# kohjingyu/gill

Hardware: AMD Instinct MI355X
Metric: 512x512 images/sec/node, OPT-6.7B+SD1.5 50-step (higher is better)
Workload: dtype bf16

## Files before the change

gill_amd/csrc/attention.hip:

```cpp
#include "ops.h"
#include <stdlib.h>
#include <type_traits>

#define ATT_KVT 64

template <int DP, int ATT_THREADS>
struct AttCfg {
  static constexpr int KS = DP / 16;
  static constexpr int NDT = (DP + 31) / 32;
  static constexpr int DPV = NDT * 32;
  static constexpr int KSTR = DP + 8;
  static constexpr int VSTR = ATT_KVT + 8;
  static constexpr bool HAS_ONES = (DP % 32) != 0;
  static constexpr int K_CHUNKS = ATT_KVT * DP / 8;
  static constexpr int V_CHUNKS = DPV * ATT_KVT / 8;
  static constexpr int K_PER_THR = (K_CHUNKS + ATT_THREADS - 1) / ATT_THREADS;
  static constexpr int V_PER_THR = (V_CHUNKS + ATT_THREADS - 1) / ATT_THREADS;
  static constexpr int K_ROWS = (K_PER_THR * ATT_THREADS + DP / 8 - 1) / (DP / 8);
  static constexpr int V_ROWS = K_PER_THR * 0 + V_PER_THR * ATT_THREADS / 8;
  static constexpr int K_ELEMS = K_ROWS * KSTR;
  static constexpr int V_ELEMS = V_ROWS * VSTR;
  static constexpr int BUF_ELEMS = K_ELEMS + V_ELEMS;
  static constexpr int SMEM_BYTES = 2 * BUF_ELEMS * 2;
};

template <int DP, int ATT_THREADS>
__global__ __launch_bounds__(ATT_THREADS, (DP <= 64 ? 4 : 2)) void attention_kernel(const AttnArgs p) {
  kernarg_warm<sizeof(AttnArgs)>();
  using Cfg = AttCfg<DP, ATT_THREADS>;
  constexpr int ATT_QB = ATT_THREADS / 2;
  constexpr int KS = Cfg::KS, NDT = Cfg::NDT, KSTR = Cfg::KSTR, VSTR = Cfg::VSTR;
  extern __shared__ __attribute__((aligned(16))) unsigned char att_smem_raw[];
  bf16_t* smem = reinterpret_cast<bf16_t*>(att_smem_raw);

  const int tid = threadIdx.x;
  const int lane = tid & 63;
  const int w = tid >> 6;
  const int nqt = (p.nq + ATT_QB - 1) / ATT_QB;
  int pair, qtile;
  if (p.xcd_map) {
    const int xcd = blockIdx.x & 7, slot = blockIdx.x >> 3;
    pair = xcd + 8 * (slot / nqt);
    qtile = slot - (slot / nqt) * nqt;
  } else {
    pair = blockIdx.x / nqt;
    qtile = blockIdx.x - pair * nqt;
  }
  if (pair >= p.B * p.H) return;
  const int b = pair / p.H, h = pair - b * p.H;
  const int q0 = qtile * ATT_QB + w * 32;
  const bool wave_active = q0 < p.nq;
  const int lq = lane & 31;
  const int hi = lane >> 5;
  const int kvb = p.kv_bstride_zero ? 0 : b;

  const bf16_t* Qb = p.Q + (size_t)(b * p.H + h) * p.nq_pad * DP;
  const bf16_t* Kb = p.K + (size_t)(kvb * p.H + h) * p.nkv_pad * DP;
  const bf16_t* Vb = p.Vt + (size_t)(kvb * p.H + h) * p.dpv * p.nkv_pad;

  int qrow = q0 + lq;
  const bool qvalid = qrow < p.nq;
  if (qrow > p.nq - 1) qrow = p.nq - 1;

  bf16x8 qf[KS];
#pragma unroll
  for (int s = 0; s < KS; ++s) qf[s] = *reinterpret_cast<const bf16x8*>(Qb + (size_t)qrow * DP + s * 16 + hi * 8);

  f32x16 oacc[NDT];
#pragma unroll
  for (int t = 0; t < NDT; ++t)
#pragma unroll
    for (int r = 0; r < 16; ++r) oacc[t][r] = 0.f;

  float m_run = 0.f, l_run = 0.f;

  const int coff = p.nkv - p.nq;
  int kv_end_blk = p.nkv;
  if (p.causal) {
    int lim = qtile * ATT_QB + ATT_QB - 1 + coff + 1;
    if (lim < kv_end_blk) kv_end_blk = lim;
    if (kv_end_blk < 1) kv_end_blk = 1;
  }
  const int ntiles = (kv_end_blk + ATT_KVT - 1) / ATT_KVT;
  const int qidx = qrow + coff;
  const int wave_kv_end = p.causal ? min(p.nkv, q0 + 31 + coff + 1) : p.nkv;

  typedef __attribute__((ext_vector_type(4))) unsigned int u32x4;
  u32x4 kreg[Cfg::K_PER_THR];
  u32x4 vreg[Cfg::V_PER_THR];
  auto gload = [&](int tile) {
    const int kv0 = tile * ATT_KVT;
#pragma unroll
    for (int i = 0; i < Cfg::K_PER_THR; ++i) {
      int c = tid + i * ATT_THREADS;
      if (c > Cfg::K_CHUNKS - 1) c = Cfg::K_CHUNKS - 1;
      int row = c / (DP / 8);
      const int col = c - row * (DP / 8);
      if (kv0 + row > p.nkv_pad - 1) row = p.nkv_pad - 1 - kv0;
      kreg[i] = *reinterpret_cast<const u32x4*>(Kb + (size_t)(kv0 + row) * DP + col * 8);
    }
#pragma unroll
    for (int i = 0; i < Cfg::V_PER_THR; ++i) {
      int c = tid + i * ATT_THREADS;
      if (c > Cfg::V_CHUNKS - 1) c = Cfg::V_CHUNKS - 1;
      const int row = c >> 3;
      int col = (c & 7) * 8;
      if (kv0 + col > p.nkv_pad - 8) col = p.nkv_pad - 8 - kv0;
      vreg[i] = *reinterpret_cast<const u32x4*>(Vb + (size_t)row * p.nkv_pad + kv0 + col);
    }
  };
  auto lstore = [&](int buf) {
    bf16_t* Ks = smem + buf * Cfg::BUF_ELEMS;
    bf16_t* Vs = Ks + Cfg::K_ELEMS;
#pragma unroll
    for (int i = 0; i < Cfg::K_PER_THR; ++i) {
      const int c = tid + i * ATT_THREADS;
      const int row = c / (DP / 8);
      const int col = c - row * (DP / 8);
      *reinterpret_cast<u32x4*>(Ks + row * KSTR + col * 8) = kreg[i];
    }
#pragma unroll
    for (int i = 0; i < Cfg::V_PER_THR; ++i) {
      const int c = tid + i * ATT_THREADS;
      const int row = c >> 3;
      const int col = (c & 7) * 8;
      bf16_t* d = Vs + row * VSTR + (col & ~15) + ((col & 8) >> 1);
      *reinterpret_cast<uint2*>(d) = make_uint2(vreg[i][0], vreg[i][1]);
      *reinterpret_cast<uint2*>(d + 8) = make_uint2(vreg[i][2], vreg[i][3]);
    }
  };

  const int rot = (p.causal || !p.xcd_map) ? 0 : (qtile * 5) % ntiles;
  gload(rot);
  lstore(0);
  __syncthreads();

  for (int it = 0; it < ntiles; ++it) {
    int tile = it + rot;
    if (tile >= ntiles) tile -= ntiles;
    const int kv0 = tile * ATT_KVT;
    if (it + 1 < ntiles) gload(tile + 1 < ntiles ? tile + 1 : 0);
    const bf16_t* Ks = smem + (it & 1) * Cfg::BUF_ELEMS;
    const bf16_t* Vs = Ks + Cfg::K_ELEMS;

    if (wave_active && kv0 < wave_kv_end) {
      const bool first = (it == 0);
      const float acc0 = first ? 0.f : -m_run;
      f32x16 s[2];
#pragma unroll
      for (int hh = 0; hh < 2; ++hh) {
#pragma unroll
        for (int r = 0; r < 16; ++r) s[hh][r] = acc0;
        const bf16_t* krow = Ks + (hh * 32 + lq) * KSTR + hi * 8;
#pragma unroll
        for (int ks = 0; ks < KS; ++ks) {
          const bf16x8 kf = *reinterpret_cast<const bf16x8*>(krow + ks * 16);
          s[hh] = __builtin_amdgcn_mfma_f32_32x32x16_bf16(kf, qf[ks], s[hh], 0, 0, 0);
        }
      }
      const bool need_mask = (kv0 + ATT_KVT > p.nkv) || (p.causal && (kv0 + ATT_KVT - 1 > q0 + coff));
      if (need_mask) {
#pragma unroll
        for (int hh = 0; hh < 2; ++hh)
#pragma unroll
          for (int r = 0; r < 16; ++r) {
            const int kv = kv0 + hh * 32 + (r & 3) + 8 * (r >> 2) + 4 * hi;
            const bool masked = (kv >= p.nkv) || (p.causal && kv > qidx);
            s[hh][r] = masked ? -INFINITY : s[hh][r];
          }
      }
      float mx = s[0][0];
#pragma unroll
      for (int hh = 0; hh < 2; ++hh)
#pragma unroll
        for (int r = 0; r < 16; ++r) mx = fmaxf(mx, s[hh][r]);
      mx = fmaxf(mx, __shfl_xor(mx, 32, 64));
      const bool grow = first || (mx > 8.0f);
      if (__any(grow)) {
        float delta;
        if (first) { m_run = (mx > -INFINITY) ? mx : 0.f; delta = m_run; }
        else { delta = grow ? mx : 0.f; m_run += delta; }
        if (!first) {
          const float alpha = __builtin_amdgcn_exp2f(-delta);
          l_run *= alpha;
#pragma unroll
          for (int t = 0; t < NDT; ++t)
#pragma unroll
            for (int r = 0; r < 16; ++r) oacc[t][r] *= alpha;
        }
#pragma unroll
        for (int hh = 0; hh < 2; ++hh)
#pragma unroll
          for (int r = 0; r < 16; ++r) s[hh][r] -= delta;
      }
#pragma unroll
      for (int hh = 0; hh < 2; ++hh)
#pragma unroll
        for (int r = 0; r < 16; ++r) s[hh][r] = __builtin_amdgcn_exp2f(s[hh][r]);
      if constexpr (!Cfg::HAS_ONES) {
        float rs = 0.f;
#pragma unroll
        for (int hh = 0; hh < 2; ++hh)
#pragma unroll
          for (int r = 0; r < 16; ++r) rs += s[hh][r];
        rs += __shfl_xor(rs, 32, 64);
        l_run += rs;
      }

      bf16x8 pa[4];
#pragma unroll
      for (int h4 = 0; h4 < 4; ++h4) {
        union { bf16x8 v; uint32_t u[4]; } pk;
#pragma unroll
        for (int j = 0; j < 4; ++j) pk.u[j] = pack_bf2(s[h4 >> 1][(h4 & 1) * 8 + 2 * j], s[h4 >> 1][(h4 & 1) * 8 + 2 * j + 1]);
        pa[h4] = pk.v;
      }
#pragma unroll
      for (int t = 0; t < NDT; ++t) {
        const bf16_t* vrow = Vs + (t * 32 + lq) * VSTR + 8 * hi;
#pragma unroll
        for (int h4 = 0; h4 < 4; ++h4) {
          const bf16x8 vf = *reinterpret_cast<const bf16x8*>(vrow + 16 * h4);
          oacc[t] = __builtin_amdgcn_mfma_f32_32x32x16_bf16(vf, pa[h4], oacc[t], 0, 0, 0);
        }
      }
    }
    if (it + 1 < ntiles) lstore((it + 1) & 1);
    __syncthreads();
  }

  if (!wave_active) return;
  if constexpr (Cfg::HAS_ONES) {
    static_assert(DP % 32 == 16, "ones-row position");
    l_run = __shfl(oacc[DP / 32][8], lq, 64);
  }
  if (!qvalid) return;
  const float inv = 1.f / l_run;
  bf16_t* orow = p.O + (size_t)(b * p.nq + qrow) * p.ldo + h * DP;
#pragma unroll
  for (int t = 0; t < NDT; ++t) {
#pragma unroll
    for (int g = 0; g < 4; ++g) {
      const int d = t * 32 + 8 * g + 4 * hi;
      if (d < DP) {
        uint2 o;
        o.x = pack_bf2(oacc[t][g * 4 + 0] * inv, oacc[t][g * 4 + 1] * inv);
        o.y = pack_bf2(oacc[t][g * 4 + 2] * inv, oacc[t][g * 4 + 3] * inv);
        *reinterpret_cast<uint2*>(orow + d) = o;
      }
    }
  }
}


template <int DP, int ATT_THREADS>
__global__ __launch_bounds__(ATT_THREADS, 4) void attention_dma_kernel(const AttnArgs p) {
  kernarg_warm<sizeof(AttnArgs)>();
  static_assert(DP == 48, "QF3 needs three padding dims behind d = 40");
  constexpr int NW = ATT_THREADS / 64;
  constexpr int ATT_QB = ATT_THREADS / 2;
  constexpr int KS = DP / 16, NDT = (DP + 31) / 32, NCH = DP / 8;
  constexpr int PPW = 8 / NW;
  constexpr int K_BYTES = 64 * 128, STAGE = 2 * K_BYTES, CONST_OFF = 2 * STAGE;
  extern __shared__ __attribute__((aligned(16))) unsigned char att_smem_raw[];
  unsigned char* smem = att_smem_raw;

  const int tid = threadIdx.x;
  const int lane = tid & 63;
  const int w = __builtin_amdgcn_readfirstlane(tid >> 6);
  const int nqt = p.nq / ATT_QB;
  int pair, qtile;
  if (p.xcd_map) {
    const int xcd = blockIdx.x & 7, slot = blockIdx.x >> 3;
    pair = xcd + 8 * (slot / nqt);
    qtile = slot - (slot / nqt) * nqt;
  } else {
    pair = blockIdx.x / nqt;
    qtile = blockIdx.x - pair * nqt;
  }
  if (pair >= p.B * p.H) return;
  const int b = pair / p.H, h = pair - b * p.H;
  const int q0 = qtile * ATT_QB + w * 32;
  const int lq = lane & 31;
  const int hi = lane >> 5;
  const int kvb = p.kv_bstride_zero ? 0 : b;

  const bf16_t* Qb = p.Q + (size_t)(b * p.H + h) * p.nq_pad * DP;
  const bf16_t* Kb = p.K + (size_t)(kvb * p.H + h) * p.nkv_pad * DP;
  const bf16_t* Vb = p.Vt + (size_t)(kvb * p.H + h) * p.dpv * p.nkv_pad;
  const int qrow = q0 + lq;

  if (tid == 0) *reinterpret_cast<uint4*>(smem + CONST_OFF) = make_uint4(0x3F803F80u, 0x00003F80u, 0u, 0u);

  bf16x8 qf[KS];
#pragma unroll
  for (int s = 0; s < KS; ++s) qf[s] = *reinterpret_cast<const bf16x8*>(Qb + (size_t)qrow * DP + s * 16 + hi * 8);

  const int r8 = lane >> 3, pch = lane & 7;
  unsigned koff[PPW], voff[PPW];
#pragma unroll
  for (int j = 0; j < PPW; ++j) {
    const int i = (w * PPW + j) * 8 + r8;
    const int c = pch ^ ((i >> 1) & 7);
    const int key = (i & ~12) | ((i & 4) << 1) | ((i & 8) >> 1);
    const int ck = c >= NCH ? c - NCH : c;
    koff[j] = (unsigned)((key * DP + ck * 8) * 2);
    voff[j] = (unsigned)((i * p.nkv_pad + c * 8) * 2);
  }
  auto issue_tile = [&](int tile, int stage) {
    const char* kbase = (const char*)(Kb + (size_t)tile * ATT_KVT * DP);
    const char* vbase = (const char*)(Vb + (size_t)tile * ATT_KVT);
    unsigned char* dst = smem + stage * STAGE + (w * PPW) * 1024;
#pragma unroll
    for (int j = 0; j < PPW; ++j) {
      __builtin_amdgcn_global_load_lds((const __attribute__((address_space(1))) void*)(kbase + koff[j]),
                                       (__attribute__((address_space(3))) void*)(dst + j * 1024), 16, 0, 0);
      __builtin_amdgcn_global_load_lds((const __attribute__((address_space(1))) void*)(vbase + voff[j]),
                                       (__attribute__((address_space(3))) void*)(dst + K_BYTES + j * 1024), 16, 0, 0);
    }
  };
  int fo[4];
#pragma unroll
  for (int c4 = 0; c4 < 4; ++c4) fo[c4] = lq * 128 + (((2 * c4 + hi) ^ ((lq >> 1) & 7)) * 16);
  int k2a[2][2];
#pragma unroll
  for (int st = 0; st < 2; ++st)
#pragma unroll
    for (int hh = 0; hh < 2; ++hh) k2a[st][hh] = hi ? CONST_OFF : st * STAGE + hh * 4096 + fo[2];

  f32x16 oacc[NDT];
#pragma unroll
  for (int t = 0; t < NDT; ++t)
#pragma unroll
    for (int r = 0; r < 16; ++r) oacc[t][r] = 0.f;
  float m_run = 0.f;

  const int ntiles = (p.nkv + ATT_KVT - 1) / ATT_KVT;
  const int rot = p.xcd_map ? (qtile * 5) % ntiles : 0;
  issue_tile(rot, 0);
  asm volatile("s_waitcnt vmcnt(0)" ::: "memory");
  __syncthreads();

  auto tile_body = [&](int it, auto stg) {
    constexpr int STG = decltype(stg)::value;
    int tile = it + rot;
    if (tile >= ntiles) tile -= ntiles;
    const int kv0 = tile * ATT_KVT;
    if (it + 1 < ntiles) issue_tile(tile + 1 < ntiles ? tile + 1 : 0, STG ^ 1);
    const unsigned char* Ks = smem + STG * STAGE;
    const unsigned char* Vs = Ks + K_BYTES;

    f32x16 s[2];
#pragma unroll
    for (int ks = 0; ks < KS; ++ks) {
#pragma unroll
      for (int hh = 0; hh < 2; ++hh) {
        const bf16x8 kf = (ks == 2) ? *reinterpret_cast<const bf16x8*>(smem + k2a[STG][hh])
                                    : *reinterpret_cast<const bf16x8*>(Ks + hh * 4096 + fo[ks]);
        if (ks == 0) s[hh] = __builtin_amdgcn_mfma_f32_32x32x16_bf16(kf, qf[ks], f32x16{0, 0, 0, 0, 0, 0, 0, 0, 0, 0, 0, 0, 0, 0, 0, 0}, 0, 0, 0);
        else s[hh] = __builtin_amdgcn_mfma_f32_32x32x16_bf16(kf, qf[ks], s[hh], 0, 0, 0);
      }
    }
    if (kv0 + ATT_KVT > p.nkv) {
#pragma unroll
      for (int hh = 0; hh < 2; ++hh)
#pragma unroll
        for (int r = 0; r < 16; ++r) {
          const int kv = kv0 + hh * 32 + 16 * (r >> 3) + 8 * hi + (r & 7);
          s[hh][r] = (kv >= p.nkv) ? -INFINITY : s[hh][r];
        }
    }
    float mx = s[0][0];
#pragma unroll
    for (int hh = 0; hh < 2; ++hh)
#pragma unroll
      for (int r = 0; r < 16; ++r) mx = fmaxf(mx, s[hh][r]);
    const bool first = (it == 0);
    if (first || __any(mx > 8.0f)) {
      mx = fmaxf(mx, __shfl_xor(mx, 32, 64));
      float delta;
      if (first) delta = (mx > -INFINITY) ? mx : 0.f;
      else delta = fmaxf(mx, 0.f);
      m_run += delta;
      {
        const float x = -m_run;
        const bf16_t a0 = f2bf(x);
        const float r1 = x - bf2f(a0);
        const bf16_t a1 = f2bf(r1);
        const float r2 = r1 - bf2f(a1);
        const bf16_t a2 = f2bf(r2);
        union { bf16x8 v; uint32_t u[4]; } xq;
        xq.v = qf[2];
        if (hi) { xq.u[0] = (uint32_t)a0 | ((uint32_t)a1 << 16); xq.u[1] = (uint32_t)a2; }
        qf[2] = xq.v;
      }
      if (!first) {
        const float alpha = __builtin_amdgcn_exp2f(-delta);
#pragma unroll
        for (int t = 0; t < NDT; ++t)
#pragma unroll
          for (int r = 0; r < 16; ++r) oacc[t][r] *= alpha;
      }
#pragma unroll
      for (int hh = 0; hh < 2; ++hh)
#pragma unroll
        for (int r = 0; r < 16; ++r) s[hh][r] -= delta;
    }
#pragma unroll
    for (int hh = 0; hh < 2; ++hh)
#pragma unroll
      for (int r = 0; r < 16; ++r) s[hh][r] = __builtin_amdgcn_exp2f(s[hh][r]);
    bf16x8 pa[4];
#pragma unroll
    for (int h4 = 0; h4 < 4; ++h4) {
      union { bf16x8 v; uint32_t u[4]; } pk;
#pragma unroll
      for (int j = 0; j < 4; ++j) pk.u[j] = pack_bf2(s[h4 >> 1][(h4 & 1) * 8 + 2 * j], s[h4 >> 1][(h4 & 1) * 8 + 2 * j + 1]);
      pa[h4] = pk.v;
    }
#pragma unroll
    for (int t = 0; t < NDT; ++t) {
#pragma unroll
      for (int h4 = 0; h4 < 4; ++h4) {
        const bf16x8 vf = *reinterpret_cast<const bf16x8*>(Vs + t * 4096 + fo[h4]);
        oacc[t] = __builtin_amdgcn_mfma_f32_32x32x16_bf16(vf, pa[h4], oacc[t], 0, 0, 0);
      }
    }
    asm volatile("s_waitcnt vmcnt(0) lgkmcnt(0)" ::: "memory");
    __builtin_amdgcn_s_barrier();
    asm volatile("" ::: "memory");
  };
  for (int it = 0; it < ntiles; it += 2) {
    tile_body(it, std::integral_constant<int, 0>{});
    if (it + 1 < ntiles) tile_body(it + 1, std::integral_constant<int, 1>{});
  }

  static_assert(DP % 32 == 16, "ones-row position");
  const float l_run = __shfl(oacc[DP / 32][8], lq, 64);
  const float inv = 1.f / l_run;
  bf16_t* orow = p.O + (size_t)(b * p.nq + qrow) * p.ldo + h * DP;
#pragma unroll
  for (int t = 0; t < NDT; ++t) {
#pragma unroll
    for (int g = 0; g < 4; ++g) {
      const int d = t * 32 + 8 * g + 4 * hi;
      if (d < DP) {
        uint2 o;
        o.x = pack_bf2(oacc[t][g * 4 + 0] * inv, oacc[t][g * 4 + 1] * inv);
        o.y = pack_bf2(oacc[t][g * 4 + 2] * inv, oacc[t][g * 4 + 3] * inv);
        *reinterpret_cast<uint2*>(orow + d) = o;
      }
    }
  }
}

template <int DP, int NTHR>
static int attention_dma_launch(const AttnArgs& a, hipStream_t s) {
  static bool attr_set = false;
  constexpr int smem = 2 * 2 * 64 * 128 + 64;
  if (!attr_set) {
    GILL_CHECK_HIP(hipFuncSetAttribute((const void*)attention_dma_kernel<DP, NTHR>, hipFuncAttributeMaxDynamicSharedMemorySize, smem));
    attr_set = true;
  }
  constexpr int xcd_on = 1;
  AttnArgs b = a;
  b.xcd_map = xcd_on;
  dim3 grid((xcd_on ? 8 * cdiv(a.H * a.B, 8) : a.H * a.B) * (a.nq / (NTHR / 2)), 1, 1);
  hipLaunchKernelGGL((attention_dma_kernel<DP, NTHR>), grid, dim3(NTHR), smem, s, b);
  GILL_CHECK_HIP(hipGetLastError());
  return 0;
}
static bool attention_dma_ok(const AttnArgs& a, int nthr) {
  static const bool on = [] { const char* e = getenv("GILL_ATT_DMA"); return !(e && e[0] == '0'); }();
  return on && a.dp == 48 && a.d == 40 && !a.causal && a.nq % (nthr / 2) == 0 && a.nkv_pad % 64 == 0 && a.dpv >= 64 && a.nkv >= 1;
}

template <int DP, int NTHR>
static int attention_launch_inst(const AttnArgs& a, hipStream_t s) {
  static bool attr_set = false;
  constexpr int smem = AttCfg<DP, NTHR>::SMEM_BYTES;
  if (!attr_set) {
    GILL_CHECK_HIP(hipFuncSetAttribute((const void*)attention_kernel<DP, NTHR>, hipFuncAttributeMaxDynamicSharedMemorySize, smem));
    attr_set = true;
  }
  constexpr int xcd_on = 1;
  AttnArgs b = a;
  b.xcd_map = xcd_on;
  dim3 grid((xcd_on ? 8 * cdiv(a.H * a.B, 8) : a.H * a.B) * cdiv(a.nq, NTHR / 2), 1, 1);
  hipLaunchKernelGGL((attention_kernel<DP, NTHR>), grid, dim3(NTHR), smem, s, b);
  GILL_CHECK_HIP(hipGetLastError());
  return 0;
}

template <int DP>
static int attention_launch_dp(const AttnArgs& a, hipStream_t s) {
  const int64_t bh = (int64_t)a.H * a.B;
  const bool big = cdiv(a.nq, 256) * bh >= 256;
  if constexpr (DP == 48) {
    if (attention_dma_ok(a, big ? 512 : 256)) return big ? attention_dma_launch<DP, 512>(a, s) : attention_dma_launch<DP, 256>(a, s);
  }
  if (big) return attention_launch_inst<DP, 512>(a, s);
  return attention_launch_inst<DP, 256>(a, s);
}

int attention_launch(const AttnArgs& a, hipStream_t s) {
  GILL_REQUIRE(a.B > 0 && a.H > 0 && a.nq > 0 && a.nkv > 0, "empty attention");
  GILL_REQUIRE(a.nkv_pad % 32 == 0 && a.nkv_pad >= a.nkv, "nkv_pad must be a multiple of 32 covering nkv");
  GILL_REQUIRE(a.nq_pad >= a.nq, "nq_pad must cover nq");
  GILL_REQUIRE(a.dpv >= round_up(a.dp, 32), "dpv must cover roundup(dp, 32)");
  GILL_REQUIRE(a.ldo >= a.H * a.dp, "ldo too small");
  switch (a.dp) {
    case 48:  return attention_launch_dp<48>(a, s);
    case 64:  return attention_launch_dp<64>(a, s);
    case 80:  return attention_launch_dp<80>(a, s);
    case 128: return attention_launch_dp<128>(a, s);
    case 160: return attention_launch_dp<160>(a, s);
    default:
      gill_set_error("attention: unsupported padded head dim (supported: 48, 64, 80, 128, 160)");
      return -2;
  }
}
```

Measured before the change: 8.517.

## Use 16x16x32 MFMA for PV product to drop padded head-dim work

Replaces the 32x32x16 MFMA PV product, which padded the head dim from 48 to 64, with 16x16x32 MFMAs over three 16-wide output tiles. Probability fragments are re-laid out with permlane16_swap, and V tiles load only the 48 needed rows, with the ones-row remapped to row 40. This removes wasted MFMA work and V loads on padding rows. In exchange it adds lane permutes, a new LDS swizzle for V reads, and a new epilogue that zero-fills padding columns.

```diff
diff --git a/gill_amd/csrc/attention.hip b/gill_amd/csrc/attention.hip
--- a/gill_amd/csrc/attention.hip
+++ b/gill_amd/csrc/attention.hip
@@ -259,8 +259,9 @@
   static_assert(DP == 48, "QF3 needs three padding dims behind d = 40");
   constexpr int NW = ATT_THREADS / 64;
   constexpr int ATT_QB = ATT_THREADS / 2;
-  constexpr int KS = DP / 16, NDT = (DP + 31) / 32, NCH = DP / 8;
+  constexpr int KS = DP / 16, NT3 = DP / 16, NCH = DP / 8;
   constexpr int PPW = 8 / NW;
+  constexpr int VPC = DP / 8;
   constexpr int K_BYTES = 64 * 128, STAGE = 2 * K_BYTES, CONST_OFF = 2 * STAGE;
   extern __shared__ __attribute__((aligned(16))) unsigned char att_smem_raw[];
   unsigned char* smem = att_smem_raw;
@@ -305,7 +306,8 @@
     const int key = (i & ~12) | ((i & 4) << 1) | ((i & 8) >> 1);
     const int ck = c >= NCH ? c - NCH : c;
     koff[j] = (unsigned)((key * DP + ck * 8) * 2);
-    voff[j] = (unsigned)((i * p.nkv_pad + c * 8) * 2);
+    const int vrow = (i == 40) ? DP : i;
+    voff[j] = (unsigned)((vrow * p.nkv_pad + c * 8) * 2);
   }
   auto issue_tile = [&](int tile, int stage) {
     const char* kbase = (const char*)(Kb + (size_t)tile * ATT_KVT * DP);
@@ -315,24 +317,29 @@
     for (int j = 0; j < PPW; ++j) {
       __builtin_amdgcn_global_load_lds((const __attribute__((address_space(1))) void*)(kbase + koff[j]),
                                        (__attribute__((address_space(3))) void*)(dst + j * 1024), 16, 0, 0);
-      __builtin_amdgcn_global_load_lds((const __attribute__((address_space(1))) void*)(vbase + voff[j]),
-                                       (__attribute__((address_space(3))) void*)(dst + K_BYTES + j * 1024), 16, 0, 0);
+      if (w * PPW + j < VPC)
+        __builtin_amdgcn_global_load_lds((const __attribute__((address_space(1))) void*)(vbase + voff[j]),
+                                         (__attribute__((address_space(3))) void*)(dst + K_BYTES + j * 1024), 16, 0, 0);
     }
   };
-  int fo[4];
-#pragma unroll
-  for (int c4 = 0; c4 < 4; ++c4) fo[c4] = lq * 128 + (((2 * c4 + hi) ^ ((lq >> 1) & 7)) * 16);
+  int fo[KS];
+#pragma unroll
+  for (int c4 = 0; c4 < KS; ++c4) fo[c4] = lq * 128 + (((2 * c4 + hi) ^ ((lq >> 1) & 7)) * 16);
+  const int m16 = lane & 15, g4 = lane >> 4;
+  int vfo[2];
+#pragma unroll
+  for (int hh = 0; hh < 2; ++hh) vfo[hh] = m16 * 128 + (((4 * hh + ((g4 & 1) << 1 | (g4 >> 1))) ^ (m16 >> 1)) * 16);
   int k2a[2][2];
 #pragma unroll
   for (int st = 0; st < 2; ++st)
 #pragma unroll
     for (int hh = 0; hh < 2; ++hh) k2a[st][hh] = hi ? CONST_OFF : st * STAGE + hh * 4096 + fo[2];
 
-  f32x16 oacc[NDT];
-#pragma unroll
-  for (int t = 0; t < NDT; ++t)
-#pragma unroll
-    for (int r = 0; r < 16; ++r) oacc[t][r] = 0.f;
+  f32x4 oacc[NT3][2];
+#pragma unroll
+  for (int t = 0; t < NT3; ++t)
+#pragma unroll
+    for (int qb = 0; qb < 2; ++qb) oacc[t][qb] = f32x4{0.f, 0.f, 0.f, 0.f};
   float m_run = 0.f;
 
   const int ntiles = (p.nkv + ATT_KVT - 1) / ATT_KVT;
@@ -396,10 +403,15 @@
       }
       if (!first) {
         const float alpha = __builtin_amdgcn_exp2f(-delta);
-#pragma unroll
-        for (int t = 0; t < NDT; ++t)
-#pragma unroll
-          for (int r = 0; r < 16; ++r) oacc[t][r] *= alpha;
+        const auto ax = __builtin_amdgcn_permlane16_swap(__float_as_uint(alpha), __float_as_uint(alpha), false, false);
+#pragma unroll
+        for (int qb = 0; qb < 2; ++qb) {
+          const float aq = __uint_as_float(ax[qb]);
+#pragma unroll
+          for (int t = 0; t < NT3; ++t)
+#pragma unroll
+            for (int r = 0; r < 4; ++r) oacc[t][qb][r] *= aq;
+        }
       }
 #pragma unroll
       for (int hh = 0; hh < 2; ++hh)
@@ -418,12 +430,28 @@
       for (int j = 0; j < 4; ++j) pk.u[j] = pack_bf2(s[h4 >> 1][(h4 & 1) * 8 + 2 * j], s[h4 >> 1][(h4 & 1) * 8 + 2 * j + 1]);
       pa[h4] = pk.v;
     }
-#pragma unroll
-    for (int t = 0; t < NDT; ++t) {
-#pragma unroll
-      for (int h4 = 0; h4 < 4; ++h4) {
-        const bf16x8 vf = *reinterpret_cast<const bf16x8*>(Vs + t * 4096 + fo[h4]);
-        oacc[t] = __builtin_amdgcn_mfma_f32_32x32x16_bf16(vf, pa[h4], oacc[t], 0, 0, 0);
+    bf16x8 pb[2][2];
+#pragma unroll
+    for (int hh = 0; hh < 2; ++hh) {
+      union { bf16x8 v; uint32_t u[4]; } x0, x1, y0, y1;
+      x0.v = pa[2 * hh];
+      x1.v = pa[2 * hh + 1];
+#pragma unroll
+      for (int j = 0; j < 4; ++j) {
+        const auto sw = __builtin_amdgcn_permlane16_swap(x0.u[j], x1.u[j], false, false);
+        y0.u[j] = sw[0];
+        y1.u[j] = sw[1];
+      }
+      pb[hh][0] = y0.v;
+      pb[hh][1] = y1.v;
+    }
+#pragma unroll
+    for (int hh = 0; hh < 2; ++hh) {
+#pragma unroll
+      for (int t = 0; t < NT3; ++t) {
+        const bf16x8 vf = *reinterpret_cast<const bf16x8*>(Vs + t * 2048 + vfo[hh]);
+#pragma unroll
+        for (int qb = 0; qb < 2; ++qb) oacc[t][qb] = __builtin_amdgcn_mfma_f32_16x16x32_bf16(vf, pb[hh][qb], oacc[t][qb], 0, 0, 0);
       }
     }
     asm volatile("s_waitcnt vmcnt(0) lgkmcnt(0)" ::: "memory");
@@ -435,21 +463,19 @@
     if (it + 1 < ntiles) tile_body(it + 1, std::integral_constant<int, 1>{});
   }
 
-  static_assert(DP % 32 == 16, "ones-row position");
-  const float l_run = __shfl(oacc[DP / 32][8], lq, 64);
-  const float inv = 1.f / l_run;
-  bf16_t* orow = p.O + (size_t)(b * p.nq + qrow) * p.ldo + h * DP;
-#pragma unroll
-  for (int t = 0; t < NDT; ++t) {
-#pragma unroll
-    for (int g = 0; g < 4; ++g) {
-      const int d = t * 32 + 8 * g + 4 * hi;
-      if (d < DP) {
-        uint2 o;
-        o.x = pack_bf2(oacc[t][g * 4 + 0] * inv, oacc[t][g * 4 + 1] * inv);
-        o.y = pack_bf2(oacc[t][g * 4 + 2] * inv, oacc[t][g * 4 + 3] * inv);
-        *reinterpret_cast<uint2*>(orow + d) = o;
-      }
+  static_assert(DP == 48, "ones-row position");
+#pragma unroll
+  for (int qb = 0; qb < 2; ++qb) {
+    const float l_run = __shfl(oacc[2][qb][0], 32 + m16, 64);
+    const float inv = 1.f / l_run;
+    bf16_t* orow = p.O + (size_t)(b * p.nq + q0 + 16 * qb + m16) * p.ldo + h * DP + 4 * g4;
+#pragma unroll
+    for (int t = 0; t < NT3; ++t) {
+      uint2 o;
+      o.x = pack_bf2(oacc[t][qb][0] * inv, oacc[t][qb][1] * inv);
+      o.y = pack_bf2(oacc[t][qb][2] * inv, oacc[t][qb][3] * inv);
+      if (t == 2 && g4 >= 2) o = make_uint2(0u, 0u);
+      *reinterpret_cast<uint2*>(orow + 16 * t) = o;
     }
   }
 }
```

Measured after the change: 8.603 (median of 6 runs). 1.0% higher.
